# lukedan/libfluid

Measured on AMD Instinct MI355X. Metric: particle_steps_per_sec, higher is better.
Workload: dtype f32

## Files before the change

### libfluid_amd/csrc/common.h

```cpp
#pragma once

#include <hip/hip_runtime.h>
#include <stdint.h>

#include <string>
#include <vector>

#include "../../include/libfluid_amd.h"

hipError_t lfa_pool_malloc(void **p, size_t bytes);
hipError_t lfa_pool_free(void *p);
void lfa_pool_nosync_begin();
void lfa_pool_nosync_end();
template <typename T> inline hipError_t lfa_hip_malloc(T **p, size_t bytes) { return lfa_pool_malloc((void **)p, bytes); }
#define hipMalloc(p, n) lfa_hip_malloc((p), (n))
#define hipFree(p) lfa_pool_free((void *)(p))
struct lfa_stream_set;
lfa_stream_set *lfa_pool_take_set(int device);
void lfa_pool_park_set(lfa_stream_set *q);

#define LFA_TILE 8
#define LFA_TILE_CELLS 512
#define LFA_HALO 10
#define LFA_HALO_CELLS 1000
#define LFA_WAVE 64

#define CT_AIR 1
#define CT_FLUID 2
#define CT_SOLID 4
#define CT_OUTSIDE 0x80

#define AB_UNKNOWN 0x40
#define AB_FLUID 0x80

struct ParticleSoA {
	uint32_t *key = nullptr;
	float *t[3] = {nullptr, nullptr, nullptr};
	float *v[3] = {nullptr, nullptr, nullptr};
	float *c[9] = {nullptr};
	uint32_t *id = nullptr;
	void *base = nullptr;
};

#define LFA_CLOSED_MAX_UNKNOWNS 64

struct GridDims {
	int nx, ny, nz;
	int ntx, nty, ntz;
	int nt;
};

struct lfa_knobs {
	int mg_no_persist = 0;
	int mg_dist_single = 0;
	int mg_co_fault = 0;
	int mg_no_top = 0;
	int mg_no_prune = 0;
	int mg_dist_levels = 0;
	int mg_no_closed = 0;
	int mg_no_tagged = 0;
};

struct lfa_sim {
	int device = 0;
	lfa_knobs knobs;
	hipStream_t stream = nullptr;
	hipStream_t stream2 = nullptr;
	hipEvent_t ev_fork = nullptr, ev_join = nullptr;
	hipStream_t stream3 = nullptr;
	hipEvent_t ev_cfork = nullptr, ev_cjoin = nullptr;
	bool overlap_correction = true;
	bool corr_in_flight = false;
	bool counts_fresh = false;
	bool move_pending = false;
	bool corr_begun = false;
	bool corr_undo_valid = false;
	uint32_t *corr_ovf = nullptr;
	int corr_parts_tiles = 0;
	GridDims g{};
	size_t nc = 0, ncp = 0;
	lfa_params prm{};
	std::string err;

	size_t np = 0, pcap = 0;
	ParticleSoA pb[2];
	int cur = 0;
	uint32_t *rank = nullptr;
	bool binned = false;

	struct lfa_dist *dist = nullptr;
	int slab_lo = 0, slab_hi = 0;
	int slab_align = 0;
	int *ptiles_all = nullptr;
	int p_off = 0, n_ptiles_all = 0;
	int n_own_first = 0, n_own_last = 0;
	int n_ghost_lo = 0, n_ghost_hi = 0;
	int *halo_tiles = nullptr;
	int n_halo[4] = {0, 0, 0, 0};
	void *xbuf[4] = {nullptr, nullptr, nullptr, nullptr};
	size_t xcap[4] = {0, 0, 0, 0};
	double *dist_red = nullptr;
	size_t np_live = 0;
	bool holes = false;
	size_t arrivals_at = 0, n_arrivals = 0;
	size_t ghost_at[2] = {0, 0}, n_ghost_particles = 0;

	uint32_t *tile_count = nullptr, *tile_start = nullptr;
	uint32_t *tile_flag = nullptr, *tile_scan = nullptr;
	uint32_t *grid_flag = nullptr;
	int *ptiles = nullptr, *dtiles = nullptr;
	int *tile_pslot = nullptr;
	int n_ptiles = 0, n_dtiles = 0;
	uint32_t *scan_tmp = nullptr;
	size_t scan_tmp_len = 0;
	uint32_t *h_pinned = nullptr;

	float *u = nullptr, *v = nullptr, *w = nullptr;
	float *uo = nullptr, *vo = nullptr, *wo = nullptr;
	uint8_t *ctype = nullptr, *solid = nullptr;
	uint32_t *cell_count = nullptr;
	uint32_t *fine_start = nullptr;
// ... 291 lines not shown
```

### libfluid_amd/csrc/core.hip

```cpp
#include <math.h>

#include <algorithm>
#include <stdarg.h>
#include <stdio.h>
#include <string.h>

#include <mutex>

#include "common.h"
#include "pcg.h"
#include "stream_set.h"

static thread_local std::string g_create_error;

int lfa_fail(lfa_sim *s, int code, const char *fmt, ...) {
	char buf[512];
	va_list ap;
	va_start(ap, fmt);
	vsnprintf(buf, sizeof buf, fmt, ap);
	va_end(ap);
	if (s) s->err = buf;
	else g_create_error = buf;
	return code;
}
// ... 142 lines not shown
	p->max_iterations = 200;
	p->p2g_variant = LFA_P2G_LDS_BINNED;
	p->precond = LFA_PRECOND_MULTIGRID;
	p->pcg_dtype = LFA_PCG_F32;
	p->apic_unscaled_kernel = 1;
	p->pcg_fused = 1;
	p->pcg_warm_start = 0;
}

template <typename T> static int dev_alloc(lfa_sim *s, T **p, size_t count, bool zero) {
	*p = nullptr;
	if (count == 0) count = 1;
	hipError_t e = hipMalloc((void **)p, count * sizeof(T));
	if (e != hipSuccess)
		return lfa_fail(s, LFA_E_OOM, "hipMalloc of %zu bytes failed: %s", count * sizeof(T), hipGetErrorString(e));
	if (zero) LFA_HIP(s, hipMemsetAsync(*p, 0, count * sizeof(T), s->stream));
	return LFA_OK;
}

__global__ void k_init_ctype(uint8_t *ctype, uint8_t *solid, GridDims g, size_t ncp) {
	size_t b = (size_t)blockIdx.x * blockDim.x + threadIdx.x;
	if (b >= ncp) return;
	int tile = (int)(b >> 9), l = (int)(b & 511), tx, ty, tz;
	tile_coords(g, tile, tx, ty, tz);
	bool in = in_grid(g, tx * 8 + (l & 7), ty * 8 + ((l >> 3) & 7), tz * 8 + (l >> 6));
	ctype[b] = in ? CT_AIR : (CT_SOLID | CT_OUTSIDE);
	solid[b] = in ? 0 : 1;
}

static hipError_t create_low_priority_stream(hipStream_t *st) {
	int least = 0, greatest = 0;
	if (hipDeviceGetStreamPriorityRange(&least, &greatest) != hipSuccess) least = 0;
	return hipStreamCreateWithPriority(st, hipStreamNonBlocking, least);
}

int lfa_pcg_grid_cap = 768;
static void lfa_knobs_parse(lfa_knobs &k) {
	auto flag = [](const char *name, int dflt) -> int {
		const char *e = getenv(name);
		return e ? (atoi(e) != 0 ? 1 : 0) : dflt;
	};
	auto num = [](const char *name, int dflt) -> int {
		const char *e = getenv(name);
		return e ? atoi(e) : dflt;
	};
	k.mg_no_persist = flag("LFA_MG_NO_PERSIST", 0);
	k.mg_dist_single = flag("LFA_MG_DIST_SINGLE", 0);
	k.mg_co_fault = num("LFA_MG_CO_FAULT", 0);
	k.mg_no_tagged = flag("LFA_MG_NO_TAGGED", 0);
	k.mg_no_top = flag("LFA_MG_NO_TOP", 0);
	k.mg_no_prune = flag("LFA_MG_NO_PRUNE", 0);
	k.mg_no_closed = flag("LFA_MG_NO_CLOSED", 0);
	k.mg_dist_levels = num("LFA_MG_DIST_LEVELS", 0);
	{
		static std::once_flag once;
		std::call_once(once, [&] {
			const int cap = num("LFA_PCG_GRID_CAP", lfa_pcg_grid_cap);
			lfa_pcg_grid_cap = cap < 1 ? 1 : (cap > 2048 ? 2048 : cap);
		});
	}
}

extern "C" int lfa_create(lfa_sim **out, uint64_t nx, uint64_t ny, uint64_t nz, int device) {
	if (!out) return lfa_fail(nullptr, LFA_E_INVALID, "lfa_create: out is NULL");
	*out = nullptr;
	if (nx == 0 || ny == 0 || nz == 0 || nx > 4096 || ny > 4096 || nz > 4096)
		return lfa_fail(nullptr, LFA_E_INVALID, "lfa_create: grid size %llux%llux%llu out of range",
		                (unsigned long long)nx, (unsigned long long)ny, (unsigned long long)nz);
	int ndev = 0;
	if (hipGetDeviceCount(&ndev) != hipSuccess || ndev == 0)
		return lfa_fail(nullptr, LFA_E_NO_DEVICE, "lfa_create: no HIP device available (there is no CPU fallback)");
	if (device < 0) {
		if (hipGetDevice(&device) != hipSuccess) device = 0;
	}
	if (device >= ndev) return lfa_fail(nullptr, LFA_E_NO_DEVICE, "lfa_create: device %d of %d", device, ndev);
	if (hipSetDevice(device) != hipSuccess) return lfa_fail(nullptr, LFA_E_NO_DEVICE, "hipSetDevice(%d) failed", device);

	lfa_sim *s = new lfa_sim();
	s->device = device;
	lfa_knobs_parse(s->knobs);
	GridDims &g = s->g;
	g.nx = (int)nx; g.ny = (int)ny; g.nz = (int)nz;
	g.ntx = (g.nx + 7) / 8; g.nty = (g.ny + 7) / 8; g.ntz = (g.nz + 7) / 8;
	g.nt = g.ntx * g.nty * g.ntz;
	s->nc = (size_t)nx * ny * nz;
	s->ncp = (size_t)g.nt * LFA_TILE_CELLS;
	if (s->ncp >= ((size_t)1 << 32)) {
		delete s;
		return lfa_fail(nullptr, LFA_E_INVALID, "lfa_create: more than 2^32 padded cells");
	}
	lfa_default_params(&s->prm);
	int rc = LFA_OK;
	auto chk = [&](int r) { if (rc == LFA_OK && r != LFA_OK) rc = r; };
	if (lfa_stream_set *q = lfa_pool_take_set(device)) {
		s->stream = q->stream; s->stream2 = q->stream2; s->stream3 = q->stream3;
		s->ev_fork = q->ev_fork; s->ev_join = q->ev_join; s->ev_cfork = q->ev_cfork; s->ev_cjoin = q->ev_cjoin;
		for (int i = 0; i < 48; ++i) s->ev[i] = q->ev[i];
		s->ev_created = q->ev_created;
		s->h_pinned = q->h_pinned;
		delete q;
	} else {
		if (hipStreamCreateWithFlags(&s->stream, hipStreamNonBlocking) != hipSuccess) {
			delete s;
			return lfa_fail(nullptr, LFA_E_HIP, "hipStreamCreate failed");
		}
		if (hipStreamCreateWithFlags(&s->stream2, hipStreamNonBlocking) != hipSuccess ||
// ... 1196 lines not shown
```

### libfluid_amd/csrc/grid_ops.hip

```cpp
#include "common.h"
#include "pcg.h"

namespace {

struct GridView {
	GridDims g;
	const uint8_t *ctype, *solid;
	const uint32_t *cell_count, *tile_flag;
};
__device__ inline bool is_unknown_at(const GridView &gv, int x, int y, int z) {
	if (!in_grid(gv.g, x, y, z)) return false;
	uint32_t b = blocked_index(gv.g, x, y, z);
	return gv.tile_flag[b >> 9] && gv.cell_count[b] > 0;
}

#define HT_UNKNOWN 8
__device__ inline void stage_halo_types(const GridView &gv, int tx, int ty, int tz, uint8_t *H) {
	for (int i = threadIdx.x; i < LFA_HALO_CELLS; i += 256) {
		const int x = 8 * tx + i % 10 - 1, y = 8 * ty + (i / 10) % 10 - 1, z = 8 * tz + i / 100 - 1;
		uint8_t t = CT_SOLID;
		if (in_grid(gv.g, x, y, z)) {
			const uint32_t b = blocked_index(gv.g, x, y, z);
			if (gv.tile_flag[b >> 9]) t = (uint8_t)((gv.ctype[b] & 7) | (gv.cell_count[b] > 0 ? HT_UNKNOWN : 0));
			else t = gv.solid[b] ? CT_SOLID : CT_AIR;
// ... 358 lines not shown
	if (threadIdx.x == 0) base = atomicAdd(n_leavers, mine < blockDim.x ? mine : blockDim.x);
	__syncthreads();
	if (i < count) leavers[base + threadIdx.x] = first + i;
}

template <int METHOD>
__global__ void __launch_bounds__(256)
k_g2p_leavers(GridDims g, ParticleSoA p, const float *u, const float *v, const float *w, const float *uo, const float *vo,
              const float *wo, G2PParams gp, const uint32_t *leavers, const uint32_t *n_leavers, ParticleSoA pold, const uint32_t *from,
              uint32_t *vmax2_bits) {
	const uint32_t n = *n_leavers;
	float vmax2 = 0.0f;
	for (uint32_t k = blockIdx.x * 256 + threadIdx.x; k < n; k += gridDim.x * 256) {
		const uint32_t i = leavers[k], key = p.key[i];
		if (key == 0xFFFFFFFFu) continue;
		const int tile = (int)(key >> 9), l = (int)(key & 511);
		int tx, ty, tz;
		tile_coords(g, tile, tx, ty, tz);
		const int cx = tx * 8 + (l & 7), cy = ty * 8 + ((l >> 3) & 7), cz = tz * 8 + (l >> 6);
		const float *F[6] = {u, v, w, uo, vo, wo};
		const float v2 = g2p_particle<METHOD>(
		    p, i, pold, (METHOD == LFA_FLIP_BLEND && from) ? from[i] : i, gp,
		    [&](int b0, int b1, int b2) { return make_int3(cx + b0, cy + b1, cz + b2); },
		    [&](int field, int comp, int3 c, int k) { return clamped_sample(g, F[field], comp, c.x + (k & 1), c.y + ((k >> 1) & 1), c.z + (k >> 2)); });
		vmax2 = fmaxf(vmax2, v2);
	}
	vmax2 = wave_max(vmax2);
	if ((threadIdx.x & 63) == 0 && vmax2 > 0.0f) atomicMax(vmax2_bits, __float_as_uint(vmax2));
}
}

static int grid_blocks(int n) { return n < 16384 ? (n > 0 ? n : 1) : 16384; }

int lfa_dist_refresh_grid(lfa_sim *s, bool with_topology) {
	if (!s->dist) return LFA_OK;
	void *f[9];
	int e[9], n = 0;
	f[n] = s->u; e[n++] = 4;
	f[n] = s->v; e[n++] = 4;
	f[n] = s->w; e[n++] = 4;
	if (with_topology) {
		f[n] = s->ctype; e[n++] = 1;
		f[n] = s->cell_count; e[n++] = 4;
		if (s->prm.simulation_method == LFA_FLIP_BLEND && s->uo) {
			f[n] = s->uo; e[n++] = 4;
			f[n] = s->vo; e[n++] = 4;
			f[n] = s->wo; e[n++] = 4;
		}
	}
	return lfa_dist_exchange_fields(s, n, f, e);
}
static GridView make_view(lfa_sim *s) { return GridView{s->g, s->ctype, s->solid, s->cell_count, s->tile_flag}; }

int lfa_build_rhs(lfa_sim *s, double dt) {
	if (!s->binned) return lfa_fail(s, LFA_E_INVALID, "lfa_build_system: call lfa_hash_particles first");
	LFA_TRY(lfa_pcg_alloc(s));
	LFA_TRY(lfa_dist_refresh_grid(s, true));
	s->a_scale = dt / (s->prm.density * s->prm.cell_size * s->prm.cell_size);
	s->sys_dt = dt;
	if (!s->n_ptiles) return LFA_OK;
	GridView gv = make_view(s);
	if (!s->tile_closed) {
		LFA_HIP(s, hipMalloc(&s->tile_closed, (size_t)s->g.nt));
		LFA_HIP(s, hipMemsetAsync(s->tile_closed, 0, (size_t)s->g.nt, s->stream));
	}
	hipLaunchKernelGGL(k_abits, dim3(grid_blocks(s->n_ptiles)), dim3(256), 0, s->stream, s->ptiles, s->n_ptiles, gv,
	                   s->abits, s->tile_closed);
	LFA_LAUNCH_CHECK(s);
	const int G = pcg_grid_uncapped(s->n_ptiles);
	const float inv_h = (float)(1.0 / s->prm.cell_size);
	if (!s->tile_epoch) {
		LFA_HIP(s, hipMalloc(&s->tile_epoch, (size_t)s->g.nt * 4));
		LFA_HIP(s, hipMemsetAsync(s->tile_epoch, 0, (size_t)s->g.nt * 4, s->stream));
	}
	s->warm_started = s->prm.pcg_warm_start && s->prm.precond != LFA_PRECOND_MIC0_EXACT && !s->dist && s->pressure_epoch == s->solve_epoch &&
	                  s->solve_epoch != 0;
	const uint32_t keep_epoch = s->warm_started ? s->solve_epoch : 0u;
	++s->solve_epoch;
	if (s->solve_epoch == 0) s->solve_epoch = 1;
	if (s->prm.pcg_dtype == LFA_PCG_F64)
		hipLaunchKernelGGL(k_rhs<double>, dim3(G), dim3(256), 0, s->stream, s->ptiles, s->n_ptiles, gv, s->u, s->v, s->w,
		                   (double *)s->vr, (double *)s->vp, inv_h, s->partials + PART_B2, s->tile_epoch, keep_epoch, s->solve_epoch);
	else
		hipLaunchKernelGGL(k_rhs<float>, dim3(G), dim3(256), 0, s->stream, s->ptiles, s->n_ptiles, gv, s->u, s->v, s->w,
		                   (float *)s->vr, (float *)s->vp, inv_h, s->partials + PART_B2, s->tile_epoch, keep_epoch, s->solve_epoch);
	LFA_LAUNCH_CHECK(s);
	return LFA_OK;
}

extern "C" int lfa_apply_pressure(lfa_sim *s, double dt) {
	if (!s) return LFA_E_INVALID;
	if (!s->binned || !s->vp) return lfa_fail(s, LFA_E_INVALID, "lfa_apply_pressure: no pressure on the device");
	LFA_HIP(s, hipSetDevice(s->device));
	if (s->dist) LFA_TRY(lfa_dist_exchange_slices(s, s->vp, s->prm.pcg_dtype == LFA_PCG_F64 ? 8 : 4));
	if (!s->n_dtiles) return LFA_OK;
	const float coeff = (float)(dt / (s->prm.density * s->prm.cell_size));
	GridView gv = make_view(s);
	dim3 grid(grid_blocks(s->n_dtiles));
	if (s->prm.pcg_dtype == LFA_PCG_F64)
		hipLaunchKernelGGL(k_apply_pressure<double>, grid, dim3(256), 0, s->stream, s->dtiles, s->n_dtiles, gv, s->u, s->v,
		                   s->w, (const double *)s->vp, coeff);
	else
		hipLaunchKernelGGL(k_apply_pressure<float>, grid, dim3(256), 0, s->stream, s->dtiles, s->n_dtiles, gv, s->u, s->v,
		                   s->w, (const float *)s->vp, coeff);
	LFA_LAUNCH_CHECK(s);
	return LFA_OK;
}

extern "C" int lfa_extrapolate(lfa_sim *s) {
	if (!s) return LFA_E_INVALID;
	if (!s->binned) return lfa_fail(s, LFA_E_INVALID, "lfa_extrapolate: call lfa_hash_particles first");
	LFA_HIP(s, hipSetDevice(s->device));
	const int iters = (int)s->prm.velocity_extrapolation_iterations;
	if (iters == 0) return LFA_OK;
	LFA_TRY(lfa_dist_refresh_grid(s, false));
	if (!s->n_dtiles) return LFA_OK;
	GridView gv = make_view(s);
	dim3 grid(grid_blocks(s->n_dtiles));
	if (iters == 1) {
		hipLaunchKernelGGL(k_extrapolate, grid, dim3(256), 0, s->stream, s->dtiles, s->n_dtiles, gv, s->u, s->v, s->w,
		                   (const uint8_t *)nullptr, (uint8_t *)nullptr);
// ... 73 lines not shown
```

### libfluid_amd/csrc/mg.hip

```cpp
#include <mutex>

#include "pcg.h"

#include <limits.h>
#include <math.h>
#include <stdio.h>
#include <stdlib.h>

#include <algorithm>
#include <vector>

#define MG_MAX_LEVELS 12
#define MG_NBR_STRIDE 8
#ifndef MG_INNER_SWEEPS
#define MG_INNER_SWEEPS 2
#endif
#define MG_OMEGA 1.15

struct lfa_mg_level {
	GridDims g{};
	size_t ncp = 0;
	int n_tiles = 0;
	int *tiles = nullptr;
	int *nbr = nullptr;
// ... 1929 lines not shown
	lfa_sim *s;
	bool on = false;
	int rc = LFA_OK;
	explicit CoGateScope(lfa_sim *s_) : g(g_co_gate[s_->device & 63]), s(s_) {
		g.m.lock();
		on = g.handles > 1;
		if (!on) {
			g.m.unlock();
			return;
		}
		for (hipEvent_t &e : g.ev)
			if (!e && hipEventCreateWithFlags(&e, hipEventDisableTiming) != hipSuccess) rc = LFA_E_HIP;
		if (rc == LFA_OK && g.n > 0 && hipStreamWaitEvent(s->stream, g.ev[(g.n - 1) & 1], 0) != hipSuccess) rc = LFA_E_HIP;
	}
	int done() {
		if (!on) return rc;
		if (rc == LFA_OK && hipEventRecord(g.ev[g.n & 1], s->stream) != hipSuccess) rc = LFA_E_HIP;
		++g.n;
		on = false;
		g.m.unlock();
		return rc;
	}
	~CoGateScope() {
		if (on) g.m.unlock();
	}
};
}
void lfa_co_gate_handle(int device, int delta) {
	CoGate &g = g_co_gate[device & 63];
	std::lock_guard<std::mutex> lk(g.m);
	g.handles += delta;
}

void lfa_mg_free(lfa_sim *s) {
	if (!s->mg) return;
	for (auto &L : s->mg->lv) {
		void *ptrs[] = {L.tiles, L.nbr, L.ctype, L.abits, L.x, L.b, L.y, L.flag, L.prev_flag, L.ready, L.xq};
		for (void *p : ptrs)
			if (p) (void)hipFree(p);
	}
	if (s->mg->l1_dirty) (void)hipFree(s->mg->l1_dirty);
	if (s->mg->l1_has_fluid) (void)hipFree(s->mg->l1_has_fluid);
	if (s->mg->slot0) (void)hipFree(s->mg->slot0);
	if (s->mg->top_ring) (void)hipFree(s->mg->top_ring);
	if (s->mg->top_buf) (void)hipFree(s->mg->top_buf);
	if (s->mg->counts) (void)hipFree(s->mg->counts);
	delete s->mg;
	s->mg = nullptr;
}

template <typename real> static int mg_setup_t(lfa_sim *s) {
	if (!s->mg) s->mg = new lfa_mg();
	lfa_mg &M = *s->mg;
	std::vector<GridDims> gs{s->g};
	while ((gs.back().nx > 8 || gs.back().ny > 8 || gs.back().nz > 8) && (int)gs.size() < MG_MAX_LEVELS) {
		GridDims c, f = gs.back();
		c.nx = (f.nx + 1) / 2; c.ny = (f.ny + 1) / 2; c.nz = (f.nz + 1) / 2;
		c.ntx = (c.nx + 7) / 8; c.nty = (c.ny + 7) / 8; c.ntz = (c.nz + 7) / 8;
		c.nt = c.ntx * c.nty * c.ntz;
		gs.push_back(c);
	}
	const int nl = (int)gs.size();
	const bool dist = mg_dist(s);
	const int d_max = s->knobs.mg_dist_levels > 0 ? std::min(s->knobs.mg_dist_levels, MG_DIST_MAX) : MG_DIST_MAX;
	const int D = dist ? std::min({d_max, s->slab_align + 1, nl - 1}) : 0;
	if (dist && D < 1) return lfa_fail(s, LFA_E_INVALID, "multigrid on slabs needs at least two levels");
	const bool realloc_all = M.n_levels != nl || M.elem != sizeof(real) || M.n_dist != D ||
	                         (nl > 1 && (M.lv[1].g.nx != gs[1].nx || M.lv[1].g.ny != gs[1].ny || M.lv[1].g.nz != gs[1].nz));
	if (realloc_all) {
		LFA_HIP(s, hipStreamSynchronize(s->stream));
		for (auto &L : M.lv) {
			void *ptrs[] = {L.tiles, L.nbr, L.ctype, L.abits, L.x, L.b, L.y, L.flag, L.prev_flag, L.ready, L.xq};
			for (void *p : ptrs)
				if (p) LFA_HIP(s, hipFree(p));
			L = lfa_mg_level();
		}
		M.n_levels = nl;
		M.elem = sizeof(real);
		M.n_dist = D;
		M.top_packed = dist && s->knobs.mg_dist_levels > 0;
		M.host_tiles.clear();
		M.host_top.clear();
		if (M.l1_dirty) LFA_HIP(s, hipFree(M.l1_dirty));
		M.l1_dirty = nullptr;
		M.solid_epoch = 0;
		if (nl > 1) LFA_HIP(s, hipMalloc(&M.l1_dirty, (size_t)gs[1].nt));
		if (M.l1_has_fluid) LFA_HIP(s, hipFree(M.l1_has_fluid));
		M.l1_has_fluid = nullptr;
		if (M.slot0) LFA_HIP(s, hipFree(M.slot0));
		M.slot0 = nullptr;
		if (nl > 1) {
			LFA_HIP(s, hipMalloc(&M.l1_has_fluid, (size_t)gs[1].nt));
			LFA_HIP(s, hipMemsetAsync(M.l1_has_fluid, 0, (size_t)gs[1].nt, s->stream));
		}
		if (!M.counts) LFA_HIP(s, hipMalloc(&M.counts, MG_MAX_LEVELS * 4));
		for (int l = 0; l < nl; ++l) {
			lfa_mg_level &L = M.lv[l];
			L.g = gs[l];
			L.ncp = (size_t)gs[l].nt * 512;
			if (!dist) {
				LFA_HIP(s, hipMalloc(&L.flag, (size_t)(gs[l].nt + 1) * 4));
				LFA_HIP(s, hipMalloc(&L.prev_flag, (size_t)(gs[l].nt + 1) * 4));
				LFA_HIP(s, hipMemsetAsync(L.prev_flag, 0, (size_t)(gs[l].nt + 1) * 4, s->stream));
				LFA_HIP(s, hipMalloc(&L.tiles, (size_t)gs[l].nt * 4));
				LFA_HIP(s, hipMalloc(&L.nbr, (size_t)gs[l].nt * MG_NBR_STRIDE * 4));
				L.cap_tiles = (size_t)gs[l].nt;
// ... 721 lines not shown
```

### libfluid_amd/csrc/p2g.hip

```cpp
#include "common.h"

namespace {

__device__ inline void axis_bf(float t, bool own, int &b, float &f) {
	if (own) {
		b = t >= 1.0f ? 0 : -1;
		f = t >= 1.0f ? 0.0f : t;
	} else {
		b = t < 0.5f ? -1 : 0;
		f = t < 0.5f ? t + 0.5f : t - 0.5f;
	}
}

template <bool APIC, bool QUIRK, typename AddFn>
__device__ inline void scatter_particle(int lx, int ly, int lz, const float t[3], const float v[3], const float c[9],
                                        float hworld, int rot, AddFn add) {
	if (QUIRK) {
#pragma unroll
		for (int comp = 0; comp < 3; ++comp) {
			float w1[3][3], a1[3][3];
			const float *cc = c + 3 * comp;
#pragma unroll
			for (int a = 0; a < 3; ++a)
#pragma unroll
// ... 149 lines not shown
			cur = nxt;
		}
		__syncthreads();
		float *out = stage + (size_t)slot * 6 * LFA_HALO_CELLS;
		for (int k = threadIdx.x; k < 6 * LFA_HALO_CELLS; k += P2G_THREADS) {
			const int ch = k / LFA_HALO_CELLS;
			out[k] = (float)((double)(long long)acc[ch * LFA_HALO_CELLS + lfa_stage_source(k - ch * LFA_HALO_CELLS)] *
			                 ((ch & 1) ? 1.0 / P2G_FIX_SCALE_W : 1.0 / P2G_FIX_SCALE_V));
		}
		__syncthreads();
	}
}

__global__ void k_zero_acc(const int *dtiles, int n_dtiles, float *acc, size_t ncp) {
	int slot = blockIdx.x;
	if (slot >= n_dtiles) return;
	size_t base = (size_t)dtiles[slot] * LFA_TILE_CELLS;
	for (int k = 0; k < 6; ++k) {
		acc[k * ncp + base + threadIdx.x] = 0.0f;
		acc[k * ncp + base + 256 + threadIdx.x] = 0.0f;
	}
}

template <bool APIC, bool QUIRK>
__global__ void __launch_bounds__(256)
k_p2g_atomic(size_t n, ParticleSoA p, float *acc, size_t ncp, GridDims g, float hworld) {
	size_t i = (size_t)blockIdx.x * blockDim.x + threadIdx.x;
	if (i >= n) return;
	const uint32_t key = p.key[i];
	const int tile = (int)(key >> 9), l = (int)(key & 511);
	int tx, ty, tz;
	tile_coords(g, tile, tx, ty, tz);
	const int cx = tx * 8 + (l & 7), cy = ty * 8 + ((l >> 3) & 7), cz = tz * 8 + (l >> 6);
	float t[3] = {p.t[0][i], p.t[1][i], p.t[2][i]};
	float v[3] = {p.v[0][i], p.v[1][i], p.v[2][i]};
	float c[9];
	if (APIC) {
#pragma unroll
		for (int k = 0; k < 9; ++k) c[k] = p.c[k][i];
	}
	scatter_particle<APIC, QUIRK>(0, 0, 0, t, v, c, hworld, 0, [&](int comp, int hx, int hy, int hz, float wv, float wgt) {
		int x = cx + hx - 1, y = cy + hy - 1, z = cz + hz - 1;
		if (!in_grid(g, x, y, z)) return;
		size_t b = blocked_index(g, x, y, z);
		unsafeAtomicAdd(acc + (size_t)(2 * comp) * ncp + b, wv);
		unsafeAtomicAdd(acc + (size_t)(2 * comp + 1) * ncp + b, wgt);
	});
}

struct FinalizeParams {
	int method;
	float g[3];
	int fuse_gravity;
};

template <bool BINNED>
__global__ void __launch_bounds__(256)
k_p2g_finalize(const int *dtiles, int n_dtiles, GridDims g, const int *tile_pslot, const float *stage, const float *acc,
               size_t ncp, const uint32_t *cell_count, const uint8_t *solid, float *u, float *v, float *w, float *uo,
               float *vo, float *wo, uint8_t *ctype, FinalizeParams fp) {
	__shared__ int ps27[27];
	for (int slot = blockIdx.x; slot < n_dtiles; slot += gridDim.x) {
		const int tile = dtiles[slot];
		int tx, ty, tz;
		tile_coords(g, tile, tx, ty, tz);
		if (BINNED) {
			__syncthreads();
			if (threadIdx.x < 27) {
				const int nx_ = tx + (int)threadIdx.x % 3 - 1, ny_ = ty + ((int)threadIdx.x / 3) % 3 - 1, nz_ = tz + (int)threadIdx.x / 9 - 1;
				const bool in = (unsigned)nx_ < (unsigned)g.ntx && (unsigned)ny_ < (unsigned)g.nty && (unsigned)nz_ < (unsigned)g.ntz;
				ps27[threadIdx.x] = in ? tile_pslot[nx_ + g.ntx * (ny_ + g.nty * nz_)] : -1;
			}
			__syncthreads();
		}
#pragma unroll
		for (int half = 0; half < 2; ++half) {
			const int l = threadIdx.x + 256 * half;
			const int lx = l & 7, ly = (l >> 3) & 7, lz = l >> 6;
			const size_t b = (size_t)tile * LFA_TILE_CELLS + l;
			const int x = tx * 8 + lx, y = ty * 8 + ly, z = tz * 8 + lz;
			float s[6] = {0.f, 0.f, 0.f, 0.f, 0.f, 0.f};
			if (BINNED) {
				const int ox0 = lx == 0 ? -1 : 0, ox1 = lx == 7 ? 1 : 0, oy0 = ly == 0 ? -1 : 0, oy1 = ly == 7 ? 1 : 0;
				const int oz0 = lz == 0 ? -1 : 0, oz1 = lz == 7 ? 1 : 0;
				for (int oz = oz0; oz <= oz1; ++oz)
					for (int oy = oy0; oy <= oy1; ++oy)
						for (int ox = ox0; ox <= ox1; ++ox) {
							const int ps = ps27[(ox + 1) + 3 * (oy + 1) + 9 * (oz + 1)];
							if (ps < 0) continue;
							const float *src = stage + (size_t)ps * 6 * LFA_HALO_CELLS + lfa_stage_index(lx - 8 * ox + 1, ly - 8 * oy + 1, lz - 8 * oz + 1);
#pragma unroll
							for (int k = 0; k < 6; ++k) s[k] += src[k * LFA_HALO_CELLS];
						}
			} else {
#pragma unroll
				for (int k = 0; k < 6; ++k) s[k] = acc[(size_t)k * ncp + b];
			}
			const bool inside = in_grid(g, x, y, z);
			float vel[3];
#pragma unroll
			for (int k = 0; k < 3; ++k) vel[k] = s[2 * k + 1] > 1e-6f ? s[2 * k] / s[2 * k + 1] : 0.0f;
			uint8_t type;
			if (!inside) {
				vel[0] = vel[1] = vel[2] = 0.0f;
				type = CT_SOLID | CT_OUTSIDE;
			} else if (solid[b]) {
				type = CT_SOLID;
			} else {
				type = cell_count[b] > 0 ? CT_FLUID : CT_AIR;
			}
			const bool bx = x == g.nx - 1, by = y == g.ny - 1, bz = z == g.nz - 1;
			if (fp.method == LFA_FLIP_BLEND && inside) {
				uo[b] = bx ? 0.0f : vel[0];
				vo[b] = by ? 0.0f : vel[1];
				wo[b] = bz ? 0.0f : vel[2];
			}
			if (fp.method == LFA_APIC) {
				if (bx) vel[0] = 0.0f;
				if (by) vel[1] = 0.0f;
				if (bz) vel[2] = 0.0f;
			}
			if (fp.fuse_gravity && inside) {
				vel[0] += fp.g[0]; vel[1] += fp.g[1]; vel[2] += fp.g[2];
			}
			u[b] = vel[0]; v[b] = vel[1]; w[b] = vel[2];
			ctype[b] = type;
		}
	}
}

__global__ void __launch_bounds__(256)
k_add_gravity(const int *dtiles, int n_dtiles, GridDims g, float *u, float *v, float *w, float gx, float gy, float gz) {
	for (int slot = blockIdx.x; slot < n_dtiles; slot += gridDim.x) {
		const int tile = dtiles[slot];
		int tx, ty, tz;
		tile_coords(g, tile, tx, ty, tz);
#pragma unroll
		for (int half = 0; half < 2; ++half) {
			const int l = threadIdx.x + 256 * half;
			if (!in_grid(g, tx * 8 + (l & 7), ty * 8 + ((l >> 3) & 7), tz * 8 + (l >> 6))) continue;
			const size_t b = (size_t)tile * LFA_TILE_CELLS + l;
			u[b] += gx; v[b] += gy; w[b] += gz;
		}
	}
}
}

static int grid_blocks(int n) { return n < 16384 ? (n > 0 ? n : 1) : 16384; }

static int scatter_mode(const lfa_sim *s) {
	if (s->prm.simulation_method != LFA_APIC) return 0;
	return (s->prm.apic_unscaled_kernel && s->prm.cell_size != 1.0) ? 2 : 1;
}
static void launch_binned(lfa_sim *s, const ParticleSoA &p, const ParticleSoA &pvc, const uint32_t *from, float *stage_own) {
	const dim3 grid(grid_blocks(s->n_ptiles));
	const float hworld = (float)s->prm.cell_size;
#define LB(A, Q)                                                                                                             \
	hipLaunchKernelGGL((k_p2g_binned<A, Q>), grid, dim3(P2G_THREADS), 0, s->stream, s->ptiles, s->n_ptiles, p, pvc, from, s->tile_start, \
	                   stage_own, hworld, rot_mask)
	const int rot_mask = 7;
	switch (scatter_mode(s)) {
	case 0: LB(false, false); break;
	case 1: LB(true, false); break;
	default: LB(true, true); break;
	}
#undef LB
}
static void launch_atomic(lfa_sim *s, const ParticleSoA &p) {
	const dim3 grid((unsigned)((s->np_live + 255) / 256));
	const float hworld = (float)s->prm.cell_size;
#define LA(A, Q) hipLaunchKernelGGL((k_p2g_atomic<A, Q>), grid, dim3(256), 0, s->stream, s->np_live, p, s->acc, s->ncp, s->g, hworld)
	switch (scatter_mode(s)) {
	case 0: LA(false, false); break;
	case 1: LA(true, false); break;
	default: LA(true, true); break;
	}
#undef LA
}

int lfa_p2g_run(lfa_sim *s, bool fuse_gravity, double dt) {
	if (!s->binned) return lfa_fail(s, LFA_E_INVALID, "lfa_p2g: call lfa_hash_particles first");
	LFA_HIP(s, hipSetDevice(s->device));
	LFA_TRY(lfa_corr_commit(s));
	const int method = s->prm.simulation_method;
	if (method == LFA_FLIP_BLEND && !s->uo) {
		LFA_HIP(s, hipMalloc(&s->uo, s->ncp * 4));
		LFA_HIP(s, hipMalloc(&s->vo, s->ncp * 4));
		LFA_HIP(s, hipMalloc(&s->wo, s->ncp * 4));
		LFA_HIP(s, hipMemsetAsync(s->uo, 0, s->ncp * 4, s->stream));
		LFA_HIP(s, hipMemsetAsync(s->vo, 0, s->ncp * 4, s->stream));
		LFA_HIP(s, hipMemsetAsync(s->wo, 0, s->ncp * 4, s->stream));
	}
	const bool binned = s->prm.p2g_variant == LFA_P2G_LDS_BINNED;
	if (!binned) LFA_TRY(lfa_particles_materialize(s));
	const ParticleSoA &p = s->pb[s->cur], &pvc = s->vc_pending ? s->pb[s->cur ^ 1] : s->pb[s->cur];
	const uint32_t *from = s->vc_pending ? (const uint32_t *)s->vc_src : (const uint32_t *)nullptr;
	if (s->timing) LFA_HIP(s, hipEventRecord(s->ev[16], s->stream));
	if (binned) {
		if ((size_t)s->n_ptiles_all > s->stage_tiles) {
			if (s->stage) LFA_HIP(s, hipFree(s->stage));
			s->stage = nullptr;
			size_t want = (size_t)s->n_ptiles_all + (size_t)s->n_ptiles_all / 4 + 16;
			hipError_t e = hipMalloc(&s->stage, want * 6 * LFA_HALO_CELLS * 4);
			if (e != hipSuccess) return lfa_fail(s, LFA_E_OOM, "hipMalloc of the P2G staging slabs (%zu tiles) failed", want);
			s->stage_tiles = want;
		}
		if (s->n_ptiles) {
			launch_binned(s, p, pvc, from, s->stage + (size_t)s->p_off * 6 * LFA_HALO_CELLS);
			LFA_LAUNCH_CHECK(s);
		}
		LFA_TRY(lfa_dist_exchange_p2g_planes(s, s->stage));
	} else {
		if (s->dist) return lfa_fail(s, LFA_E_UNSUPPORTED, "the global-atomic P2G variant is single-GPU only");
		if (!s->acc) {
			hipError_t e = hipMalloc(&s->acc, s->ncp * 6 * 4);
			if (e != hipSuccess) return lfa_fail(s, LFA_E_OOM, "hipMalloc of the atomic P2G accumulators failed");
		}
		if (s->n_dtiles) {
			hipLaunchKernelGGL(k_zero_acc, dim3(s->n_dtiles), dim3(256), 0, s->stream, s->dtiles, s->n_dtiles, s->acc,
			                   s->ncp);
			LFA_LAUNCH_CHECK(s);
		}
		if (s->np_live) {
			launch_atomic(s, p);
			LFA_LAUNCH_CHECK(s);
		}
	}
	if (s->timing) LFA_HIP(s, hipEventRecord(s->ev[17], s->stream));
	FinalizeParams fp;
	fp.method = method;
	fp.fuse_gravity = fuse_gravity ? 1 : 0;
	for (int k = 0; k < 3; ++k) fp.g[k] = fuse_gravity ? (float)(s->prm.gravity[k] * dt) : 0.0f;
	if (s->n_dtiles) {
		dim3 grid(grid_blocks(s->n_dtiles));
		if (binned)
			hipLaunchKernelGGL(k_p2g_finalize<true>, grid, dim3(256), 0, s->stream, s->dtiles, s->n_dtiles, s->g,
			                   s->tile_pslot, s->stage, s->acc, s->ncp, s->cell_count, s->solid, s->u, s->v, s->w, s->uo,
			                   s->vo, s->wo, s->ctype, fp);
		else
			hipLaunchKernelGGL(k_p2g_finalize<false>, grid, dim3(256), 0, s->stream, s->dtiles, s->n_dtiles, s->g,
			                   s->tile_pslot, s->stage, s->acc, s->ncp, s->cell_count, s->solid, s->u, s->v, s->w, s->uo,
			                   s->vo, s->wo, s->ctype, fp);
		LFA_LAUNCH_CHECK(s);
	}
	LFA_HIP(s, hipMemcpyAsync(s->grid_flag, s->tile_flag, (size_t)s->g.nt * 4, hipMemcpyDeviceToDevice, s->stream));
	s->grid_valid = true;
	s->system_valid = false;
	for (int k = 0; k < 3; ++k) s->bg[k] = fuse_gravity ? s->prm.gravity[k] * dt : 0.0;
	return LFA_OK;
}

extern "C" int lfa_p2g(lfa_sim *s) {
	if (!s) return LFA_E_INVALID;
	return lfa_p2g_run(s, false, 0.0);
}

extern "C" int lfa_add_gravity(lfa_sim *s, double dt) {
	if (!s) return LFA_E_INVALID;
	LFA_HIP(s, hipSetDevice(s->device));
	if (s->binned && s->n_dtiles) {
		hipLaunchKernelGGL(k_add_gravity, dim3(grid_blocks(s->n_dtiles)), dim3(256), 0, s->stream, s->dtiles, s->n_dtiles,
		                   s->g, s->u, s->v, s->w, (float)(s->prm.gravity[0] * dt), (float)(s->prm.gravity[1] * dt),
		                   (float)(s->prm.gravity[2] * dt));
		LFA_LAUNCH_CHECK(s);
	}
	for (int k = 0; k < 3; ++k) s->bg[k] += s->prm.gravity[k] * dt;
	s->system_valid = false;
	return LFA_OK;
}

int lfa_p2g_bench(lfa_sim *s, int which) {
	if (which == LFA_K_P2G_SCATTER && s->prm.p2g_variant != LFA_P2G_LDS_BINNED) LFA_TRY(lfa_particles_materialize(s));
	const ParticleSoA &p = s->pb[s->cur], &pvc = s->vc_pending ? s->pb[s->cur ^ 1] : s->pb[s->cur];
	const uint32_t *from = s->vc_pending ? (const uint32_t *)s->vc_src : (const uint32_t *)nullptr;
	if (which == LFA_K_P2G_SCATTER) {
		if (s->prm.p2g_variant == LFA_P2G_LDS_BINNED) {
			if (!s->stage || (size_t)s->n_ptiles_all > s->stage_tiles) return lfa_fail(s, LFA_E_INVALID, "no staging slabs");
			launch_binned(s, p, pvc, from, s->stage + (size_t)s->p_off * 6 * LFA_HALO_CELLS);
		} else {
			if (!s->acc) return lfa_fail(s, LFA_E_INVALID, "no accumulators");
			launch_atomic(s, p);
		}
		LFA_LAUNCH_CHECK(s);
		return LFA_OK;
	}
	if (which == LFA_K_P2G_FINALIZE) {
		FinalizeParams fp;
		fp.method = s->prm.simulation_method;
		fp.fuse_gravity = 0;
		fp.g[0] = fp.g[1] = fp.g[2] = 0.f;
		dim3 grid(grid_blocks(s->n_dtiles));
		if (s->prm.p2g_variant == LFA_P2G_LDS_BINNED)
			hipLaunchKernelGGL(k_p2g_finalize<true>, grid, dim3(256), 0, s->stream, s->dtiles, s->n_dtiles, s->g,
			                   s->tile_pslot, s->stage, s->acc, s->ncp, s->cell_count, s->solid, s->u, s->v, s->w, s->uo,
			                   s->vo, s->wo, s->ctype, fp);
		else
			hipLaunchKernelGGL(k_p2g_finalize<false>, grid, dim3(256), 0, s->stream, s->dtiles, s->n_dtiles, s->g,
			                   s->tile_pslot, s->stage, s->acc, s->ncp, s->cell_count, s->solid, s->u, s->v, s->w, s->uo,
			                   s->vo, s->wo, s->ctype, fp);
		LFA_LAUNCH_CHECK(s);
		return LFA_OK;
	}
	if (which == LFA_K_BIN) return lfa_hash_particles(s);
	return lfa_fail(s, LFA_E_INVALID, "unknown kernel id %d", which);
}
```

### libfluid_amd/csrc/particles.hip

```cpp
#include <math.h>

#include <algorithm>
#include <utility>

#include "common.h"
#include "pcg.h"

namespace {

__device__ inline bool solid_or_outside(const GridDims &g, const uint8_t *solid, int x, int y, int z) {
	if (!in_grid(g, x, y, z)) return true;
	return solid[blocked_index(g, x, y, z)] != 0;
}

__device__ inline void collide(const GridDims &g, const uint8_t *solid, double from[3], double to[3], double skin) {
	for (int bounce = 0; bounce < 3; ++bounce) {
		bool hit = false;
		double diff[3], inv[3], t[3];
		int cur[3], last[3], adv[3];
#pragma unroll
		for (int d = 0; d < 3; ++d) {
			cur[d] = (int)floor(from[d]);
			last[d] = (int)floor(to[d]);
			diff[d] = to[d] - from[d];
// ... 1272 lines not shown
__global__ void __launch_bounds__(256)
k_correct_undo(size_t n, const float4 *spos, const uint32_t *old_key, uint32_t *key, float *t0, float *t1, float *t2) {
	const size_t k = (size_t)blockIdx.x * blockDim.x + threadIdx.x;
	if (k >= n) return;
	const float4 rec = spos[k];
	const uint32_t i = __float_as_uint(rec.w);
	t0[i] = __uint_as_float(__float_as_uint(rec.x) & 0x3FFFFFFFu);
	t1[i] = __uint_as_float(__float_as_uint(rec.y) & 0x3FFFFFFFu);
	t2[i] = __uint_as_float(__float_as_uint(rec.z) & 0x3FFFFFFFu);
	key[k] = old_key[k];
}
}

extern "C" int lfa_correct_collide_undo(lfa_sim *s) {
	if (!s) return LFA_E_INVALID;
	if (!s->corr_begun) return LFA_OK;
	if (!s->corr_undo_valid)
		return lfa_fail(s, LFA_E_INVALID, "lfa_correct_collide_undo: positions, binning or solid cells have changed since lfa_correct_collide_begin");
	LFA_HIP(s, hipSetDevice(s->device));
	LFA_TRY(lfa_corr_commit(s));
	s->corr_begun = false;
	const size_t n = s->np_live;
	if (!n) return LFA_OK;
	ParticleSoA &cur = s->pb[s->cur], &oth = s->pb[s->cur ^ 1];
	hipLaunchKernelGGL(k_correct_undo, dim3((unsigned)((n + 255) / 256)), dim3(256), 0, s->stream, n, (const float4 *)correction_scratch(s),
	                   (const uint32_t *)oth.key, cur.key, cur.t[0], cur.t[1], cur.t[2]);
	LFA_LAUNCH_CHECK(s);
	return LFA_OK;
}

int lfa_g2p_stale(lfa_sim *s);
extern "C" int lfa_time_step(lfa_sim *s, double dt, double *residual, uint64_t *iterations) {
	if (!s) return LFA_E_INVALID;
	LFA_HIP(s, hipSetDevice(s->device));
	LFA_TRY(lfa_corr_commit(s));
	const bool tm = s->timing;
	enum { B_START = 24, B_ADVECT, B_BIN, B_P2G, B_SOLVE, B_APPLY, B_CORRECT, B_EXTRAP, B_G2P, B_JOIN };
	static_assert(B_CORRECT == LFA_EV_CORRECT_END, "event slot of the end of the correction");
	auto rec = [&](int id) -> int {
		if (tm) LFA_HIP(s, hipEventRecord(s->ev[id], s->stream));
		return LFA_OK;
	};
	LFA_TRY(rec(B_START));
	LFA_TRY(advect_collide(s, dt, true));
	LFA_TRY(rec(B_ADVECT));
	{
		const bool counted = s->counts_fresh;
		s->counts_fresh = false;
		LFA_TRY(lfa_hash_particles_impl(s, counted));
	}
	if (!s->sources.empty()) LFA_TRY(lfa_update_sources(s, nullptr));
	LFA_TRY(rec(B_BIN));
	const bool overlap = s->overlap_correction && (s->dist || s->np_live);
	LFA_TRY(lfa_p2g_run(s, true, dt));
	LFA_TRY(rec(B_P2G));
	if (overlap) {
		if (s->dist) LFA_TRY(lfa_dist_exchange_ghost_particles(s));
		LFA_TRY(correct_begin(s, dt, true));
	}
	double res = 0.0;
	uint64_t it = 0;
	int rc = LFA_OK;
	auto grid_stages = [&]() -> int {
		rc = lfa_pcg_solve(s, dt, &res, &it);
		if (rc < 0) return rc;
		LFA_TRY(rec(B_SOLVE));
		LFA_TRY(lfa_apply_pressure(s, dt));
		LFA_TRY(rec(B_APPLY));
		if (!overlap) {
			LFA_TRY(lfa_correct_collide(s, dt));
			LFA_TRY(rec(B_CORRECT));
		}
		LFA_TRY(lfa_extrapolate(s));
		return rec(B_EXTRAP);
	};
	const int rc_grid = grid_stages();
	if (overlap) LFA_TRY(lfa_corr_join(s));
	if (rc_grid < 0) return rc_grid;
	if (overlap && s->dist) LFA_TRY(lfa_dist_migrate(s, true));
	LFA_TRY(rec(B_JOIN));
	LFA_TRY(lfa_g2p_stale(s));
	if (tm) {
		LFA_TRY(rec(B_G2P));
		LFA_HIP(s, hipEventSynchronize(s->ev[B_G2P]));
		auto span = [&](int a, int b, double &out) -> int {
			float ms = 0.f;
			LFA_HIP(s, hipEventElapsedTime(&ms, s->ev[a], s->ev[b]));
			out = ms;
			return LFA_OK;
		};
		double *m = s->ms_next;
		const bool solved = it || s->n_ptiles;
		LFA_TRY(span(B_START, B_ADVECT, m[0]));
		LFA_TRY(span(B_ADVECT, B_BIN, m[1]));
		LFA_TRY(span(B_BIN, B_P2G, m[2]));
		LFA_TRY(span(16, 17, m[3]));
		if (solved) {
			LFA_TRY(span(B_P2G, 18, m[4]));
			LFA_TRY(span(18, B_SOLVE, m[5]));
		} else {
			LFA_TRY(span(B_P2G, B_SOLVE, m[4]));
			m[5] = 0.0;
		}
		LFA_TRY(span(B_SOLVE, B_APPLY, m[6]));
		if (s->np_live) {
			LFA_TRY(span(40, 41, m[7]));
			LFA_TRY(span(41, 42, m[8]));
		} else {
			m[7] = m[8] = 0.0;
		}
		if (overlap && !s->np_live) {
			m[9] = 0.0;
		} else {
			LFA_TRY(span(overlap ? 40 : B_APPLY, B_CORRECT, m[9]));
		}
		LFA_TRY(span(overlap ? B_APPLY : B_CORRECT, B_EXTRAP, m[10]));
		LFA_TRY(span(B_JOIN, B_G2P, m[11]));
		m[15] = overlap ? 1.0 : 0.0;
		LFA_TRY(span(B_START, B_G2P, m[12]));
		m[13] = (double)it;
		m[14] = it ? m[5] / (double)it : 0.0;
	}
	if (residual) *residual = res;
	if (iterations) *iterations = it;
	return rc;
}

extern "C" int lfa_get_correction_stats(lfa_sim *s, uint64_t stats[2]) {
	if (!s || !stats) return LFA_E_INVALID;
// ... 37 lines not shown
```

### libfluid_amd/csrc/pcg.h

```cpp
#pragma once
#include "common.h"

#define PCG_MAX_GRID 2048
#define PCG_WAVES 4
enum { PART_STRIDE = PCG_MAX_GRID + 64, PART_ZS = 0, PART_RMAX = PART_STRIDE, PART_SIG0 = 2 * PART_STRIDE,
       PART_SIG1 = 3 * PART_STRIDE, PART_B2 = 4 * PART_STRIDE, PART_TOTAL = 5 * PART_STRIDE };

extern int lfa_pcg_grid_cap;
static inline int pcg_grid(int n_ptiles) {
	int g = (n_ptiles + PCG_WAVES - 1) / PCG_WAVES;
	if (g < 1) g = 1;
	return g < lfa_pcg_grid_cap ? g : lfa_pcg_grid_cap;
}

static inline int pcg_grid_uncapped(int n_ptiles) {
	int g = (n_ptiles + PCG_WAVES - 1) / PCG_WAVES;
	if (g < 1) g = 1;
	return g < PCG_MAX_GRID ? g : PCG_MAX_GRID;
}

int lfa_build_rhs(lfa_sim *s, double dt);
int lfa_p2g_run(lfa_sim *s, bool fuse_gravity, double dt);
int lfa_dist_refresh_grid(lfa_sim *s, bool with_topology);

int lfa_mg_setup(lfa_sim *s);
int lfa_mg_apply(lfa_sim *s, double *part_sigma);
int lfa_mg_axpy_apply(lfa_sim *s, const void *sdir, const double *part_sigma, int n_sigma, const double *part_qs, int n_qs,
                      double *part_rmax, double *part_sigma_new);
int lfa_mg_axpy_apply_cg(lfa_sim *s, const double *gamma, int n_gamma, const double *gamma_old, int n_gamma_old, const double *delta,
                         int n_delta, const double *rmax_prev, int n_rmax, int iter, double *alpha_io, double *part_rmax,
                         double *part_sigma_new);
int lfa_mg_bench_part(lfa_sim *s, int part);
int lfa_mg_level0(const lfa_sim *s, const int **tiles, const int **slot);
int lfa_mg_solve_closed(lfa_sim *s, void *out = nullptr);
void lfa_mg_free(lfa_sim *s);
void lfa_mg_stats(const lfa_sim *s, uint64_t *launches_per_cycle, uint64_t *levels, uint64_t *first_co);
```

### libfluid_amd/csrc/pcg.hip

```cpp
#include "pcg.h"

#include <math.h>
#include <string.h>

#include <stdlib.h>

#include <algorithm>

namespace {

#define WAVE_SYNC() asm volatile("s_waitcnt lgkmcnt(0)" ::: "memory")

template <typename real> struct Vecs {
	real *p, *r, *z, *s, *pre, *q;
};

struct TileCtx {
	const int *ptiles;
	int n_ptiles;
	const int *tile_pslot;
	GridDims g;
};

__device__ inline void face_neighbours(const TileCtx &tc, int tile, int nb[6]) {
// ... 1452 lines not shown
	const int G = pcg_grid(s->n_ptiles);
	if (s->prm.precond == LFA_PRECOND_MIC0_EXACT) {
		const int nl = (int)s->level_offsets.size() - 1;
		for (int l = 0; l < nl; ++l) {
			const int b = s->level_offsets[l], n = s->level_offsets[l + 1] - b;
			if (!n) continue;
			hipLaunchKernelGGL((k_mic_apply<real, SWEEP_FWD, false>), dim3((n + PCG_WAVES - 1) / PCG_WAVES), dim3(256), 0, s->stream,
			                   tc, s->level_tiles + b, n, s->abits, v, scale, part_sigma, s->pcg_state, (real *)nullptr,
			                   (const int *)nullptr, CoarseFields<real>{}, CoarseArgs{});
			LFA_LAUNCH_CHECK(s);
		}
		for (int l = nl - 1; l >= 0; --l) {
			const int b = s->level_offsets[l], n = s->level_offsets[l + 1] - b;
			if (!n) continue;
			hipLaunchKernelGGL((k_mic_apply<real, SWEEP_BWD, false>), dim3((n + PCG_WAVES - 1) / PCG_WAVES), dim3(256), 0, s->stream,
			                   tc, s->level_tiles + b, n, s->abits, v, scale, part_sigma, s->pcg_state, (real *)nullptr,
			                   (const int *)nullptr, CoarseFields<real>{}, CoarseArgs{});
			LFA_LAUNCH_CHECK(s);
		}
		hipLaunchKernelGGL(k_dot_zr<real>, dim3(G), dim3(256), 0, s->stream, tc, v, part_sigma, s->pcg_state);
		LFA_LAUNCH_CHECK(s);
	} else {
		const bool embed = is_ml(s) && r1_ready && s->n_l1tiles <= 64;
		if (embed) {
			CoarseArgs ca{s->l1_tiles, s->n_l1tiles, s->a2inv, s->c_x2, (double *)s->pcg_hist + 6144, (unsigned *)(s->pcg_state + 4)};
			hipLaunchKernelGGL((k_mic_apply<real, SWEEP_BOTH, true>), dim3(G + PCG_COARSE_BLOCKS), dim3(256), 0, s->stream, tc,
			                   (const int *)nullptr, s->n_ptiles, s->abits, v, scale, part_sigma, s->pcg_state, (real *)nullptr,
			                   (const int *)s->slot_l1, make_coarse<real>(s), ca);
			LFA_LAUNCH_CHECK(s);
		} else {
			hipLaunchKernelGGL((k_mic_apply<real, SWEEP_BOTH, false>), dim3(G), dim3(256), 0, s->stream, tc,
			                   (const int *)nullptr, s->n_ptiles, s->abits, v, scale, part_sigma, s->pcg_state,
			                   (is_ml(s) && !r1_ready) ? (real *)s->c_r : (real *)nullptr, (const int *)s->slot_l1,
			                   CoarseFields<real>{}, CoarseArgs{});
			LFA_LAUNCH_CHECK(s);
			if (is_ml(s)) LFA_TRY(coarse_apply<real>(s, part_sigma, s->stream));
		}
	}
	return LFA_OK;
}

static int pcg_scrub(lfa_sim *s) {
	LFA_HIP(s, hipStreamSynchronize(s->stream));
	lfa_mg_free(s);
	void *vs[] = {s->vp, s->vr, s->vz, s->vs, s->vpre, s->vq, s->vs2};
	for (void *v : vs)
		if (v) LFA_HIP(s, hipMemsetAsync(v, 0, s->ncp * s->vec_elem, s->stream));
	s->pressure_epoch = 0;
	s->warm_started = false;
	s->pcg_poisoned = false;
	return LFA_OK;
}

template <typename real> static int build_system_t(lfa_sim *s, double dt) {
	if (s->pcg_poisoned) LFA_TRY(pcg_scrub(s));
	LFA_TRY(lfa_build_rhs(s, dt));
	if (s->n_ptiles || (s->dist && is_mg(s))) LFA_TRY(mic_factor<real>(s));
	s->system_valid = true;
	return LFA_OK;
}

extern "C" int lfa_build_system(lfa_sim *s, double dt) {
	if (!s) return LFA_E_INVALID;
	LFA_HIP(s, hipSetDevice(s->device));
	LFA_TRY(lfa_pcg_alloc(s));
	return s->prm.pcg_dtype == LFA_PCG_F64 ? build_system_t<double>(s, dt) : build_system_t<float>(s, dt);
}

template <typename real, typename... Args>
static void launch_pcg_a(bool first, bool coarse, int grid, hipStream_t st, Args... a) {
	if (first && coarse) hipLaunchKernelGGL((k_pcg_a<real, true, true>), dim3(grid), dim3(256), 0, st, a...);
	else if (first) hipLaunchKernelGGL((k_pcg_a<real, true, false>), dim3(grid), dim3(256), 0, st, a...);
	else if (coarse) hipLaunchKernelGGL((k_pcg_a<real, false, true>), dim3(grid), dim3(256), 0, st, a...);
	else hipLaunchKernelGGL((k_pcg_a<real, false, false>), dim3(grid), dim3(256), 0, st, a...);
}

static void fused_grids(int G, int &GA, int &GB) {
	static int n_cu = 0;
	if (!n_cu) {
		int dev = 0;
		hipDeviceProp_t prop;
		n_cu = (hipGetDevice(&dev) == hipSuccess && hipGetDeviceProperties(&prop, dev) == hipSuccess &&
		        prop.multiProcessorCount > 0) ? prop.multiProcessorCount : 256;
	}
	GA = std::min(G, 4 * n_cu);
	GB = std::min(G, 8 * n_cu);
}

template <typename real> static int solve_t(lfa_sim *s, double dt, double *residual, uint64_t *iterations) {
	if (s->dist && s->prm.precond == LFA_PRECOND_MIC0_EXACT)
		return lfa_fail(s, LFA_E_UNSUPPORTED, "the exact (hyperplane) MIC(0) schedule is single-GPU only");
	LFA_TRY(build_system_t<real>(s, dt));
	if (s->timing) LFA_HIP(s, hipEventRecord(s->ev[18], s->stream));
	const int first_chunk = s->last_iters > 0 ? (int)std::min<uint64_t>(s->last_iters, 4096) : 8;
	const uint64_t calls_at_start = s->dist ? s->dist->calls : 0;
	s->stat_launches_iter = s->stat_transport_iter = s->stat_transport_solve = s->stat_mg_levels = s->stat_mg_first_co = 0;
	s->last_residual = 0.0;
	s->last_iters = 0;
	if (residual) *residual = 0.0;
	if (iterations) *iterations = 0;
	if (!s->n_ptiles && !s->dist) return LFA_OK;
	TileCtx tc = make_ctx(s);
	Vecs<real> v = make_vecs<real>(s);
	const int n_it = iter_ctx(s).n_ptiles;
	const int G = pcg_grid(n_it);
	const real scale = (real)s->a_scale;
	double *P = s->partials;
	const bool dist = s->dist != nullptr;
	int init_state[4] = {-1, 0, 0, 0};
	LFA_HIP(s, hipMemcpyAsync(s->pcg_state, init_state, 16, hipMemcpyHostToDevice, s->stream));
	const bool host_check = dist || s->last_rhs_zero;
// ... 566 lines not shown
```

Baseline: 5.008 billion.

## Overlap cell typing and pressure geometry setup with P2G on a side stream

```diff
diff --git a/libfluid_amd/csrc/common.h b/libfluid_amd/csrc/common.h
--- a/libfluid_amd/csrc/common.h
+++ b/libfluid_amd/csrc/common.h
@@ -59,6 +59,7 @@
 	int mg_dist_levels = 0;
 	int mg_no_closed = 0;
 	int mg_no_tagged = 0;
+	int no_early_setup = 0;
 };
 
 struct lfa_sim {
@@ -67,6 +68,8 @@
 	hipStream_t stream = nullptr;
 	hipStream_t stream2 = nullptr;
 	hipEvent_t ev_fork = nullptr, ev_join = nullptr;
+	bool types_early = false;
+	bool geometry_ready = false;
 	hipStream_t stream3 = nullptr;
 	hipEvent_t ev_cfork = nullptr, ev_cjoin = nullptr;
 	bool overlap_correction = true;
diff --git a/libfluid_amd/csrc/core.hip b/libfluid_amd/csrc/core.hip
--- a/libfluid_amd/csrc/core.hip
+++ b/libfluid_amd/csrc/core.hip
@@ -218,6 +218,7 @@
 	k.mg_no_prune = flag("LFA_MG_NO_PRUNE", 0);
 	k.mg_no_closed = flag("LFA_MG_NO_CLOSED", 0);
 	k.mg_dist_levels = num("LFA_MG_DIST_LEVELS", 0);
+	k.no_early_setup = flag("LFA_NO_EARLY_SETUP", 0);
 	{
 		static std::once_flag once;
 		std::call_once(once, [&] {
diff --git a/libfluid_amd/csrc/grid_ops.hip b/libfluid_amd/csrc/grid_ops.hip
--- a/libfluid_amd/csrc/grid_ops.hip
+++ b/libfluid_amd/csrc/grid_ops.hip
@@ -434,7 +434,7 @@
 }
 static GridView make_view(lfa_sim *s) { return GridView{s->g, s->ctype, s->solid, s->cell_count, s->tile_flag}; }
 
-int lfa_build_rhs(lfa_sim *s, double dt) {
+int lfa_build_geometry(lfa_sim *s, double dt) {
 	if (!s->binned) return lfa_fail(s, LFA_E_INVALID, "lfa_build_system: call lfa_hash_particles first");
 	LFA_TRY(lfa_pcg_alloc(s));
 	LFA_TRY(lfa_dist_refresh_grid(s, true));
@@ -449,6 +449,13 @@
 	hipLaunchKernelGGL(k_abits, dim3(grid_blocks(s->n_ptiles)), dim3(256), 0, s->stream, s->ptiles, s->n_ptiles, gv,
 	                   s->abits, s->tile_closed);
 	LFA_LAUNCH_CHECK(s);
+	return LFA_OK;
+}
+
+int lfa_build_rhs(lfa_sim *s, double dt) {
+	(void)dt;
+	if (!s->n_ptiles) return LFA_OK;
+	GridView gv = make_view(s);
 	const int G = pcg_grid_uncapped(s->n_ptiles);
 	const float inv_h = (float)(1.0 / s->prm.cell_size);
 	if (!s->tile_epoch) {
diff --git a/libfluid_amd/csrc/mg.hip b/libfluid_amd/csrc/mg.hip
--- a/libfluid_amd/csrc/mg.hip
+++ b/libfluid_amd/csrc/mg.hip
@@ -2005,6 +2005,7 @@
 template <typename real> static int mg_setup_t(lfa_sim *s) {
 	if (!s->mg) s->mg = new lfa_mg();
 	lfa_mg &M = *s->mg;
+	M.closed_out = false;
 	std::vector<GridDims> gs{s->g};
 	while ((gs.back().nx > 8 || gs.back().ny > 8 || gs.back().nz > 8) && (int)gs.size() < MG_MAX_LEVELS) {
 		GridDims c, f = gs.back();
diff --git a/libfluid_amd/csrc/p2g.hip b/libfluid_amd/csrc/p2g.hip
--- a/libfluid_amd/csrc/p2g.hip
+++ b/libfluid_amd/csrc/p2g.hip
@@ -225,6 +225,7 @@
 	int method;
 	float g[3];
 	int fuse_gravity;
+	int write_types;
 };
 
 template <bool BINNED>
@@ -297,6 +298,25 @@
 				vel[0] += fp.g[0]; vel[1] += fp.g[1]; vel[2] += fp.g[2];
 			}
 			u[b] = vel[0]; v[b] = vel[1]; w[b] = vel[2];
+			if (fp.write_types) ctype[b] = type;
+		}
+	}
+}
+
+__global__ void __launch_bounds__(256)
+k_cell_types(const int *dtiles, int n_dtiles, GridDims g, const uint32_t *cell_count, const uint8_t *solid, uint8_t *ctype) {
+	for (int slot = blockIdx.x; slot < n_dtiles; slot += gridDim.x) {
+		const int tile = dtiles[slot];
+		int tx, ty, tz;
+		tile_coords(g, tile, tx, ty, tz);
+#pragma unroll
+		for (int half = 0; half < 2; ++half) {
+			const int l = threadIdx.x + 256 * half;
+			const size_t b = (size_t)tile * LFA_TILE_CELLS + l;
+			uint8_t type;
+			if (!in_grid(g, tx * 8 + (l & 7), ty * 8 + ((l >> 3) & 7), tz * 8 + (l >> 6))) type = CT_SOLID | CT_OUTSIDE;
+			else if (solid[b]) type = CT_SOLID;
+			else type = cell_count[b] > 0 ? CT_FLUID : CT_AIR;
 			ctype[b] = type;
 		}
 	}
@@ -351,7 +371,18 @@
 #undef LA
 }
 
+int lfa_cell_types(lfa_sim *s) {
+	if (!s->n_dtiles) return LFA_OK;
+	hipLaunchKernelGGL(k_cell_types, dim3(grid_blocks(s->n_dtiles)), dim3(256), 0, s->stream, s->dtiles, s->n_dtiles, s->g,
+	                   s->cell_count, s->solid, s->ctype);
+	LFA_LAUNCH_CHECK(s);
+	return LFA_OK;
+}
+
 int lfa_p2g_run(lfa_sim *s, bool fuse_gravity, double dt) {
+	const bool types_early = s->types_early;
+	s->types_early = false;
+	s->geometry_ready = false;
 	if (!s->binned) return lfa_fail(s, LFA_E_INVALID, "lfa_p2g: call lfa_hash_particles first");
 	LFA_HIP(s, hipSetDevice(s->device));
 	LFA_TRY(lfa_corr_commit(s));
@@ -403,6 +434,7 @@
 	FinalizeParams fp;
 	fp.method = method;
 	fp.fuse_gravity = fuse_gravity ? 1 : 0;
+	fp.write_types = types_early ? 0 : 1;
 	for (int k = 0; k < 3; ++k) fp.g[k] = fuse_gravity ? (float)(s->prm.gravity[k] * dt) : 0.0f;
 	if (s->n_dtiles) {
 		dim3 grid(grid_blocks(s->n_dtiles));
@@ -461,6 +493,7 @@
 		FinalizeParams fp;
 		fp.method = s->prm.simulation_method;
 		fp.fuse_gravity = 0;
+		fp.write_types = 1;
 		fp.g[0] = fp.g[1] = fp.g[2] = 0.f;
 		dim3 grid(grid_blocks(s->n_dtiles));
 		if (s->prm.p2g_variant == LFA_P2G_LDS_BINNED)
diff --git a/libfluid_amd/csrc/particles.hip b/libfluid_amd/csrc/particles.hip
--- a/libfluid_amd/csrc/particles.hip
+++ b/libfluid_amd/csrc/particles.hip
@@ -1348,11 +1348,25 @@
 	if (!s->sources.empty()) LFA_TRY(lfa_update_sources(s, nullptr));
 	LFA_TRY(rec(B_BIN));
 	const bool overlap = s->overlap_correction && (s->dist || s->np_live);
-	LFA_TRY(lfa_p2g_run(s, true, dt));
+	const bool early = lfa_geometry_early_applies(s);
+	s->geometry_ready = false;
+	if (early) LFA_TRY(lfa_geometry_fork(s));
+	const int rc_p2g = lfa_p2g_run(s, true, dt);
+	s->types_early = false;
+	if (rc_p2g < 0) return rc_p2g;
 	LFA_TRY(rec(B_P2G));
+	if (early) {
+		const int rc_geo = lfa_geometry_early(s, dt);
+		LFA_TRY(lfa_geometry_join(s));
+		if (rc_geo < 0) return rc_geo;
+	}
 	if (overlap) {
 		if (s->dist) LFA_TRY(lfa_dist_exchange_ghost_particles(s));
-		LFA_TRY(correct_begin(s, dt, true));
+		const int rc_corr = correct_begin(s, dt, true);
+		if (rc_corr < 0) {
+			s->geometry_ready = false;
+			return rc_corr;
+		}
 	}
 	double res = 0.0;
 	uint64_t it = 0;
@@ -1371,6 +1385,7 @@
 		return rec(B_EXTRAP);
 	};
 	const int rc_grid = grid_stages();
+	s->geometry_ready = false;
 	if (overlap) LFA_TRY(lfa_corr_join(s));
 	if (rc_grid < 0) return rc_grid;
 	if (overlap && s->dist) LFA_TRY(lfa_dist_migrate(s, true));
diff --git a/libfluid_amd/csrc/pcg.h b/libfluid_amd/csrc/pcg.h
--- a/libfluid_amd/csrc/pcg.h
+++ b/libfluid_amd/csrc/pcg.h
@@ -19,8 +19,14 @@
 	return g < PCG_MAX_GRID ? g : PCG_MAX_GRID;
 }
 
+int lfa_build_geometry(lfa_sim *s, double dt);
 int lfa_build_rhs(lfa_sim *s, double dt);
 int lfa_p2g_run(lfa_sim *s, bool fuse_gravity, double dt);
+int lfa_cell_types(lfa_sim *s);
+bool lfa_geometry_early_applies(const lfa_sim *s);
+int lfa_geometry_fork(lfa_sim *s);
+int lfa_geometry_early(lfa_sim *s, double dt);
+int lfa_geometry_join(lfa_sim *s);
 int lfa_dist_refresh_grid(lfa_sim *s, bool with_topology);
 
 int lfa_mg_setup(lfa_sim *s);
diff --git a/libfluid_amd/csrc/pcg.hip b/libfluid_amd/csrc/pcg.hip
--- a/libfluid_amd/csrc/pcg.hip
+++ b/libfluid_amd/csrc/pcg.hip
@@ -1528,11 +1528,51 @@
 	return LFA_OK;
 }
 
+template <typename real> static int build_geometry_t(lfa_sim *s, double dt) {
+	LFA_TRY(lfa_build_geometry(s, dt));
+	if (s->n_ptiles || (s->dist && is_mg(s))) LFA_TRY(mic_factor<real>(s));
+	return LFA_OK;
+}
+
 template <typename real> static int build_system_t(lfa_sim *s, double dt) {
 	if (s->pcg_poisoned) LFA_TRY(pcg_scrub(s));
+	const bool have_geometry = s->geometry_ready && s->sys_dt == dt;
+	s->geometry_ready = false;
+	if (!have_geometry) LFA_TRY(build_geometry_t<real>(s, dt));
 	LFA_TRY(lfa_build_rhs(s, dt));
-	if (s->n_ptiles || (s->dist && is_mg(s))) LFA_TRY(mic_factor<real>(s));
 	s->system_valid = true;
+	return LFA_OK;
+}
+
+bool lfa_geometry_early_applies(const lfa_sim *s) {
+	return !s->knobs.no_early_setup && !s->dist && is_mg(s) && s->n_ptiles > 0 && s->n_dtiles > 0;
+}
+
+int lfa_geometry_fork(lfa_sim *s) {
+	s->geometry_ready = false;
+	LFA_TRY(lfa_pcg_alloc(s));
+	if (s->pcg_poisoned) LFA_TRY(pcg_scrub(s));
+	LFA_HIP(s, hipEventRecord(s->ev_fork, s->stream));
+	LFA_HIP(s, hipStreamWaitEvent(s->stream2, s->ev_fork, 0));
+	s->types_early = true;
+	return LFA_OK;
+}
+
+int lfa_geometry_early(lfa_sim *s, double dt) {
+	hipStream_t main_stream = s->stream;
+	s->stream = s->stream2;
+	int rc = lfa_cell_types(s);
+	if (rc == LFA_OK) rc = s->prm.pcg_dtype == LFA_PCG_F64 ? build_geometry_t<double>(s, dt) : build_geometry_t<float>(s, dt);
+	s->stream = main_stream;
+	const hipError_t e = hipEventRecord(s->ev_join, s->stream2);
+	if (rc < 0) return rc;
+	LFA_HIP(s, e);
+	s->geometry_ready = true;
+	return LFA_OK;
+}
+
+int lfa_geometry_join(lfa_sim *s) {
+	LFA_HIP(s, hipStreamWaitEvent(s->stream, s->ev_join, 0));
 	return LFA_OK;
 }
 
```

Result: no change. 4.995 billion (-0.3%).
